# thimabru1010/ResUnet-a_mltsk_keras

Hardware: AMD Instinct MI355X
Metric: training patches/sec (256×256, 6-ch, bs=8/GPU) at 1/2/4/8 MI355X (higher is better)
Workload: dtype bf16; 1 GPU; cfg3: ResUnet-a d6 multitask (seg+bound+dist+color) Tanimoto-dual, 256x256x6, 6 classes, Adam, full train step (fwd+loss+bwd+allreduce+update); global_batch=8, per_gpu_batch=8, parallelism=dp1

## Files before the change

### include/rua_hip.h

```cpp
#ifndef RUA_HIP_H
#define RUA_HIP_H
#include <stdint.h>
#ifdef __cplusplus
extern "C" {
#endif

#define RUA_F32 0
#define RUA_BF16 1
#define RUA_MAX_SEG 6
#define RUA_MAX_BRANCH 4
#define RUA_MAX_WGRAD_BATCH 32
#define RUA_MAX_WGRAD_GROUP 8

#define RUA_OK 0
#define RUA_ERR_ARG (-1)
#define RUA_ERR_LAUNCH (-2)

int rua_version(void);
const char* rua_last_error(void);
int rua_device_info(int* cu_count, int* lds_bytes, char* arch, int arch_len);

typedef struct rua_conv_seg {
  const void* x;
  const void* w;
// ... 10 lines not shown
  float eps, momentum;
  const float* gamma; const float* beta;
  float* moving_mean; float* moving_var;
  float* scale; float* shift; float* mean; float* rstd;
} rua_bn_fold;

typedef struct rua_conv_desc {
  rua_conv_seg seg[RUA_MAX_SEG];
  int32_t nseg;
  int32_t N, H, W, Cout;
  int32_t stride;
  int32_t dtype;
  const float* bias;
  const void* aux;
  int32_t aux_mode;
  const float* mscale;
  const float* mshift;
  int32_t out_relu;
  int32_t accumulate;
  void* y;
  int32_t out_stride, OH, OW;
  double* stats;
  int32_t stats_mode;
  void* workspace;
  int64_t workspace_bytes;
  int32_t stats_replicas;
  const float* bias_more[3];
  const float* in_scale;
  const float* in_shift;
  int32_t in_relu;
  int32_t pad_fold;
  const struct rua_bn_fold* in_fold;
} rua_conv_desc;
int rua_conv_fwd(const rua_conv_desc* d, void* stream);
int rua_conv_fwd_group(const rua_conv_desc* d, int n, void* stream);
int rua_conv_group_last_grids(void);
int rua_conv_group_band_ok(const rua_conv_desc* d, int n);
int rua_conv_group_last_band(void);
int rua_conv_group_last_chain(void);
int rua_conv_fwd_sum(const rua_conv_desc* d, int n, void* stream);
int rua_conv_sum_last_kernel(void);
int rua_conv_sum_kernel(const rua_conv_desc* d, int n);
int rua_conv_smem_bytes(const rua_conv_desc* d);
int64_t rua_conv_workspace_bytes(const rua_conv_desc* d);
void* rua_prof_event_create(void);
int rua_prof_event_record(void* ev, void* hip_stream);
int rua_prof_event_elapsed_us(void* start, void* stop, double* us);
void rua_prof_event_destroy(void* ev);
void rua_profile_mid_event(void* hip_event);
int rua_profile_mid_event_fired(void);
int rua_conv_last_ksplit(void);
int rua_conv_tile_bn(const rua_conv_desc* d);
int rua_conv_kernel_id(const rua_conv_desc* d);
int rua_conv_fused_input_ok(const rua_conv_desc* d);
int rua_conv_tile_bm(const rua_conv_desc* d);

typedef struct rua_wgrad_desc {
  const void* a;  int32_t C, Hs, Ws;
  const void* dy; int32_t Cout, H, W;
  int32_t N, stride, dil, taps, dtype;
  float* dw;
  void* workspace;
  int64_t workspace_bytes;
  const float* in_scale;
  const float* in_shift;
  int32_t in_relu;
  int32_t defer;
  int32_t group_members;
  int32_t batch;
  const int32_t* overwrite_dev;
} rua_wgrad_desc;
typedef struct rua_wgrad_pending {
  int32_t kind;
  int32_t parts;
  int64_t n;
  const float* partials;
  float* dw;
  int32_t CC;
  int32_t blocks;
  int32_t block_begin, pad;
  const int32_t* overwrite_dev;
} rua_wgrad_pending;
int rua_wgrad_plan(const rua_wgrad_desc* d, rua_wgrad_pending* out);
int rua_wgrad_reduce_batch(const rua_wgrad_pending* items_dev, int n_items, int total_blocks, void* stream);
int rua_conv_wgrad(const rua_wgrad_desc* d, void* stream);
int rua_conv_wgrad_group(const rua_wgrad_desc* d, int n, void* stream);
int rua_wgrad_group_last_grids(void);
int rua_wgrad_group_plan(const rua_wgrad_desc* d, int n, rua_wgrad_pending* out);
int64_t rua_wgrad_workspace_bytes(const rua_wgrad_desc* d);
int rua_wgrad_kind(const rua_wgrad_desc* d);
int rua_wgrad_img_kind(const rua_wgrad_desc* d);

typedef struct rua_wprep_item { int64_t src_off, dst_off; int32_t taps, Cout, C, pad; } rua_wprep_item;
int rua_weight_prep(const float* master, void* w_fwd, void* w_dgrad, const rua_wprep_item* items_dev,
                    int n_items, int max_elems, int dtype, void* stream);
int rua_weight_prep_dgrad(const void* w_fwd, void* w_dgrad, const rua_wprep_item* items_dev, int n_items, int max_elems, const int32_t* blockmap_dev,
                          int n_blocks, int dtype, void* stream);
int rua_wprep_blocks(int taps, int Cout, int C);

int rua_stem_fwd(const float* x, const float* w, const float* b, void* y, int64_t M, int Cin, int Cout, int dtype, void* stream);
int rua_stem_fwd_stats(const float* x, const float* w, const float* b, void* y, int64_t M, int Cin, int Cout, int dtype, double* stats, int replicas, void* stream);
int rua_stem_bwd(const float* x, const void* dy, float* dw, float* db, int64_t M, int Cin, int Cout, int dtype, void* stream);
int rua_stem_fwd_pack(const float* x, const float* w, const float* b, void* y, int64_t M, int Cin, int Cout, int dtype, double* stats, int replicas,
                      void* xpack, void* stream);
int rua_stem_bwd_fold(float* tmp, float* dw, float* db, int Cin, int Cout, void* stream);
int rua_head_fwd(const void* x, const float* w, const float* b, float* z, float* p, int64_t M, int Cin, int Cout, int act, int dtype, void* stream);
// ... 176 lines not shown
```

### resunet_a_mltsk_keras_amd/_lib.py

```python
from __future__ import annotations

import ctypes as C
import os

HERE = os.path.dirname(os.path.abspath(__file__))
LIB_PATH = os.environ.get("RUA_LIB_PATH") or os.path.join(HERE, "librua_hip.so")

RUA_F32, RUA_BF16 = 0, 1
RUA_MAX_SEG, RUA_MAX_BRANCH, RUA_MAX_WGRAD_GROUP, RUA_MAX_WGRAD_BATCH = 6, 4, 8, 32
LOSS_TANIMOTO, LOSS_WCE, LOSS_CE_LOGITS, LOSS_BCE_LOGITS, LOSS_MSE = 0, 1, 2, 3, 4
ACT_NONE, ACT_SOFTMAX, ACT_SIGMOID = 0, 1, 2

vp, i32, i64, f32, f64 = C.c_void_p, C.c_int32, C.c_int64, C.c_float, C.c_double


class ConvSeg(C.Structure):
    _fields_ = [("x", vp), ("w", vp), ("C", i32), ("Hs", i32), ("Ws", i32), ("up_shift", i32), ("dil", i32), ("taps", i32)]


class ConvDesc(C.Structure):
    _fields_ = [("seg", ConvSeg * RUA_MAX_SEG), ("nseg", i32), ("N", i32), ("H", i32), ("W", i32), ("Cout", i32),
                ("stride", i32), ("dtype", i32), ("bias", vp), ("aux", vp), ("aux_mode", i32), ("mscale", vp),
                ("mshift", vp), ("out_relu", i32), ("accumulate", i32), ("y", vp), ("out_stride", i32), ("OH", i32),
                ("OW", i32), ("stats", vp), ("stats_mode", i32), ("workspace", vp), ("workspace_bytes", i64), ("stats_replicas", i32),
# ... 11 lines not shown
                ("in_scale", vp), ("in_shift", vp), ("in_relu", i32), ("defer", i32), ("group_members", i32), ("batch", i32), ("overwrite_dev", vp)]


class WgradPending(C.Structure):
    _fields_ = [("kind", i32), ("parts", i32), ("n", i64), ("partials", vp), ("dw", vp), ("CC", i32), ("blocks", i32),
                ("block_begin", i32), ("pad", i32), ("overwrite_dev", vp)]


class TaniHead(C.Structure):
    _fields_ = [("sums", vp), ("replicas", i32), ("B", i32), ("C", i32), ("grad_scale", f32), ("loss_out", vp), ("coef", vp), ("per_sample", vp)]


class DzHead(C.Structure):
    _fields_ = [("kind", i32), ("act", i32), ("p", vp), ("y", vp), ("coef", vp), ("class_w", vp), ("grad_scale", f32), ("B", i32), ("HW", i64),
                ("C", i32), ("pad", i32), ("dz", vp)]


class BnBranch(C.Structure):
    _fields_ = [("gamma", vp), ("beta", vp), ("moving_mean", vp), ("moving_var", vp), ("scale", vp), ("shift", vp),
                ("mean", vp), ("rstd", vp), ("out", vp), ("stats", vp), ("replicas", i32), ("pad", i32), ("out_stats", vp)]


class BnFwdDesc(C.Structure):
    _fields_ = [("x", vp), ("M", i64), ("C", i32), ("dtype", i32), ("nb", i32), ("relu", i32), ("training", i32), ("replicas", i32),
                ("stats", vp), ("count", f64), ("bessel_n", f64), ("momentum", f32), ("eps", f32), ("br", BnBranch * RUA_MAX_BRANCH)]


class BnBwdBranch(C.Structure):
    _fields_ = [("g", vp), ("stats2", vp), ("replicas", i32), ("stats2_out", i32), ("gamma", vp), ("mean", vp), ("rstd", vp),
                ("scale", vp), ("shift", vp), ("dgamma", vp), ("dbeta", vp)]


class BnBwdDesc(C.Structure):
    _fields_ = [("x", vp), ("dskip", vp), ("dx", vp), ("M", i64), ("C", i32), ("dtype", i32), ("nb", i32), ("masked", i32),
                ("accumulate", i32), ("pad", i32), ("count", f64), ("br", BnBwdBranch * RUA_MAX_BRANCH),
                ("skip_stats", vp), ("skip_replicas", i32), ("pad2", i32), ("dx_stats", vp), ("dx_replicas", i32), ("pad3", i32)]


class WprepItem(C.Structure):
    _fields_ = [("src_off", i64), ("dst_off", i64), ("taps", i32), ("Cout", i32), ("C", i32), ("pad", i32)]


PP = C.POINTER(vp)

_SIGS = {
    "rua_version": ([], i32),
    "rua_device_info": ([C.POINTER(i32), C.POINTER(i32), C.c_char_p, i32], i32),
    "rua_conv_fwd": ([C.POINTER(ConvDesc), vp], i32),
    "rua_conv_fwd_group": ([C.POINTER(ConvDesc), i32, vp], i32),
    "rua_conv_smem_bytes": ([C.POINTER(ConvDesc)], i32),
    "rua_conv_tile_bn": ([C.POINTER(ConvDesc)], i32),
    "rua_conv_tile_bm": ([C.POINTER(ConvDesc)], i32),
    "rua_conv_kernel_id": ([C.POINTER(ConvDesc)], i32),
    "rua_conv_fused_input_ok": ([C.POINTER(ConvDesc)], i32),
    "rua_conv_last_ksplit": ([], i32),
    "rua_conv_group_last_grids": ([], i32),
    "rua_conv_group_band_ok": ([C.POINTER(ConvDesc), i32], i32),
    "rua_conv_group_last_band": ([], i32),
    "rua_conv_group_last_chain": ([], i32),
    "rua_conv_fwd_sum": ([C.POINTER(ConvDesc), i32, vp], i32),
    "rua_conv_sum_last_kernel": ([], i32),
    "rua_conv_sum_kernel": ([C.POINTER(ConvDesc), i32], i32),
    "rua_conv_wgrad_group": ([C.POINTER(WgradDesc), i32, vp], i32),
    "rua_wgrad_group_last_grids": ([], i32),
    "rua_wgrad_group_plan": ([C.POINTER(WgradDesc), i32, C.POINTER(WgradPending)], i32),
    "rua_profile_mid_event": ([vp], None),
    "rua_profile_mid_event_fired": ([], i32),
    "rua_prof_event_create": ([], vp),
    "rua_prof_event_record": ([vp, vp], i32),
    "rua_prof_event_elapsed_us": ([vp, vp, C.POINTER(f64)], i32),
    "rua_prof_event_destroy": ([vp], None),
    "rua_graph_kernel_nodes": ([vp, C.POINTER(i32), C.POINTER(i32)], i32),
    "rua_conv_workspace_bytes": ([C.POINTER(ConvDesc)], i64),
    "rua_conv_wgrad": ([C.POINTER(WgradDesc), vp], i32),
    "rua_wgrad_workspace_bytes": ([C.POINTER(WgradDesc)], i64),
    "rua_wgrad_kind": ([C.POINTER(WgradDesc)], i32),
    "rua_wgrad_img_kind": ([C.POINTER(WgradDesc)], i32),
    "rua_wgrad_plan": ([C.POINTER(WgradDesc), C.POINTER(WgradPending)], i32),
    "rua_wgrad_reduce_batch": ([vp, i32, i32, vp], i32),
    "rua_weight_prep": ([vp, vp, vp, vp, i32, i32, i32, vp], i32),
    "rua_weight_prep_dgrad": ([vp, vp, vp, i32, i32, vp, i32, i32, vp], i32),
    "rua_wprep_blocks": ([i32, i32, i32], i32),
    "rua_stem_fwd": ([vp, vp, vp, vp, i64, i32, i32, i32, vp], i32),
    "rua_stem_fwd_stats": ([vp, vp, vp, vp, i64, i32, i32, i32, vp, i32, vp], i32),
    "rua_stem_bwd": ([vp, vp, vp, vp, i64, i32, i32, i32, vp], i32),
    "rua_stem_fwd_pack": ([vp, vp, vp, vp, i64, i32, i32, i32, vp, i32, vp, vp], i32),
    "rua_stem_bwd_fold": ([vp, vp, vp, i32, i32, vp], i32),
    "rua_head_fwd": ([vp, vp, vp, vp, vp, i64, i32, i32, i32, i32, vp], i32),
    "rua_head_fwd_loss": ([vp, vp, vp, vp, vp, vp, vp, vp, i32, i64, i32, i32, i32, i32, vp], i32),
    "rua_head_fwd_loss_rep": ([vp, vp, vp, vp, vp, vp, vp, i32, vp, i32, i64, i32, i32, i32, i32, vp], i32),
    "rua_head_bwd": ([vp, vp, vp, vp, i32, vp, vp, vp, i64, i64, i32, i32, i32, i32, vp], i32),
    "rua_head_bwd_sums": ([vp, vp, vp, vp, i32, vp, vp, vp, vp, i64, i64, i32, i32, i32, i32, vp], i32),
    "rua_col_stats": ([vp, i64, i32, vp, i32, i32, vp], i32),
    "rua_col_stats2": ([vp, vp, vp, vp, i32, i64, i32, vp, i32, i32, vp], i32),
    "rua_stats_replicas": ([i64], i32),
    "rua_bn_finalize": ([vp, i32, f64, f64, vp, vp, vp, vp, f32, f32, i32, vp, vp, vp, vp, i32, vp], i32),
    "rua_bn_apply": ([vp, i32, PP, PP, i32, PP, i64, i32, i32, vp], i32),
    "rua_bn_bwd_finalize": ([vp, i32, f64, vp, vp, vp, vp, vp, vp, vp, vp, i32, vp], i32),
    "rua_bn_bwd_apply": ([i32, PP, PP, PP, PP, PP, PP, i32, vp, vp, vp, i32, i64, i32, i32, vp], i32),
    "rua_stats_to_f32": ([vp, i32, i32, PP, i32, vp], i32),
    "rua_bn_fwd": ([C.POINTER(BnFwdDesc), vp], i32),
    "rua_bn_fwd_group": ([C.POINTER(BnFwdDesc), i32, vp], i32),
    "rua_bn_fwd_group_last_grids": ([], i32),
    "rua_bn_bwd": ([C.POINTER(BnBwdDesc), vp], i32),
    "rua_bn_bwd_group": ([C.POINTER(BnBwdDesc), i32, vp], i32),
    "rua_bn_bwd_group_last_grids": ([], i32),
# ... 116 lines not shown
```

### resunet_a_mltsk_keras_amd/csrc/capi.cpp

```cpp
#include <hip/hip_runtime.h>
#include <stdarg.h>
#include <stdio.h>
#include <string.h>
#include <stdint.h>
#include "common.h"

static thread_local char g_err[512] = "";
RuaTuning g_tune;

void rua_set_error(const char* fmt, ...) {
  va_list ap;
  va_start(ap, fmt);
  vsnprintf(g_err, sizeof(g_err), fmt, ap);
  va_end(ap);
}

extern "C" const char* rua_last_error(void) { return g_err; }
extern "C" int rua_version(void) { return 200; }

extern "C" int rua_device_info(int* cu_count, int* lds_bytes, char* arch, int arch_len) {
  hipDeviceProp_t prop;
  int dev = 0;
  if (hipGetDevice(&dev) != hipSuccess || hipGetDeviceProperties(&prop, dev) != hipSuccess) {
    rua_set_error("rua_device_info: no HIP device");
// ... 41 lines not shown
  int k = 0;
  if (n && hipGraphGetNodes((hipGraph_t)graph, nodes, &n) == hipSuccess)
    for (size_t i = 0; i < n; ++i) {
      hipGraphNodeType t;
      if (hipGraphNodeGetType(nodes[i], &t) == hipSuccess && t == hipGraphNodeTypeKernel) ++k;
    }
  delete[] nodes;
  if (kernels) *kernels = k;
  if (total) *total = (int)n;
  return RUA_OK;
}

int rua_device_index() {
  int dev = 0;
  if (hipGetDevice(&dev) != hipSuccess || dev < 0) { (void)hipGetLastError(); dev = 0; }
  return dev;
}

int rua_cu_count() {
  static int cached[64] = {0};
  const int dev = rua_device_index();
  if (dev >= 64) return 256;
  if (cached[dev] == 0) {
    int n = 0;
    if (hipDeviceGetAttribute(&n, hipDeviceAttributeMultiprocessorCount, dev) != hipSuccess || n <= 0) { (void)hipGetLastError(); n = 256; }
    cached[dev] = n;
  }
  int n = cached[dev] - (g_tune.cu_reserve > 0 ? g_tune.cu_reserve : 0);
  return n < 16 ? 16 : n;
}

struct TuneKey { const char* name; int* i; long long* ll; };
static const TuneKey* tune_table(int* n) {
  static const TuneKey t[] = {
    {"conv_force_bn", &g_tune.conv_force_bn, nullptr}, {"conv_force_bm", &g_tune.conv_force_bm, nullptr}, {"conv_dma", &g_tune.conv_dma, nullptr},
    {"conv_pw", &g_tune.conv_pw, nullptr}, {"conv_pw_minm", nullptr, &g_tune.conv_pw_minm}, {"conv_pw_blocks", &g_tune.conv_pw_blocks, nullptr},
    {"conv_halo", &g_tune.conv_halo, nullptr}, {"conv_dmap", &g_tune.conv_dmap, nullptr}, {"dmap_target", &g_tune.dmap_target, nullptr},
    {"dmap_fused_finish", &g_tune.dmap_fused_finish, nullptr}, {"dmap_rowb", &g_tune.dmap_rowb, nullptr}, {"dmap_bm64", &g_tune.dmap_bm64, nullptr},
    {"wgrad_pw", &g_tune.wgrad_pw, nullptr}, {"wgpw_blocks", &g_tune.wgpw_blocks, nullptr}, {"wgpw_r", &g_tune.wgpw_r, nullptr},
    {"wgd_blocks", &g_tune.wgd_blocks, nullptr}, {"wgrad_dmap", &g_tune.wgrad_dmap, nullptr}, {"wgd_mintiles", &g_tune.wgd_mintiles, nullptr},
    {"wgrad_blocks", &g_tune.wgrad_blocks, nullptr}, {"bn_grid", &g_tune.bn_grid, nullptr}, {"tani_vec", &g_tune.tani_vec, nullptr},
    {"metrics_blocks", &g_tune.metrics_blocks, nullptr}, {"stem_blocks", &g_tune.stem_blocks, nullptr}, {"head_blocks", &g_tune.head_blocks, nullptr},
    {"conv_img", &g_tune.conv_img, nullptr}, {"conv_strip", &g_tune.conv_strip, nullptr}, {"wgrad_slabs", &g_tune.wgrad_slabs, nullptr},
    {"strip_narrow_maxd", &g_tune.strip_narrow_maxd, nullptr}, {"conv_group", &g_tune.conv_group, nullptr}, {"wgrad_group", &g_tune.wgrad_group, nullptr},
    {"wgrad_batch_blocks", &g_tune.wgrad_batch_blocks, nullptr}, {"wgd_ks_slow", &g_tune.wgd_ks_slow, nullptr}, {"head_fwd2", &g_tune.head_fwd2, nullptr},
    {"head_fwd3", &g_tune.head_fwd3, nullptr}, {"head_fwd3_bpc", &g_tune.head_fwd3_bpc, nullptr}, {"stem_reg", &g_tune.stem_reg, nullptr},
    {"stats_blocks", &g_tune.stats_blocks, nullptr}, {"conv_band", &g_tune.conv_band, nullptr}, {"conv_band64", &g_tune.conv_band64, nullptr},
    {"conv_band64m", &g_tune.conv_band64m, nullptr}, {"strip_group_share", &g_tune.strip_group_share, nullptr}, {"band_dbg", &g_tune.band_dbg, nullptr},
    {"fill_kernel", &g_tune.fill_kernel, nullptr}, {"bn_regs", &g_tune.bn_regs, nullptr}, {"wgrad_taps_share", &g_tune.wgrad_taps_share, nullptr},
    {"dmap_chain", &g_tune.dmap_chain, nullptr}, {"epi_fast", &g_tune.epi_fast, nullptr}, {"dmap_spread", &g_tune.dmap_spread, nullptr},
    {"bn_bwd_group", &g_tune.bn_bwd_group, nullptr}, {"conv_small", &g_tune.conv_small, nullptr}, {"strip_stag", &g_tune.strip_stag, nullptr},
    {"cu_reserve", &g_tune.cu_reserve, nullptr}, {"wgrad_rows", &g_tune.wgrad_rows, nullptr}, {"strip_seglen", &g_tune.strip_seglen, nullptr},
    {"band_stag", &g_tune.band_stag, nullptr}, {"conv_band128m", &g_tune.conv_band128m, nullptr}, {"conv_img2", &g_tune.conv_img2, nullptr},
    {"dbg_ptr", nullptr, &g_tune.dbg_ptr},
  };
  *n = (int)(sizeof(t) / sizeof(t[0]));
  return t;
}
extern "C" int rua_set_tuning(const char* key, int64_t value) {
  int n; const TuneKey* t = tune_table(&n);
  for (int i = 0; key && i < n; ++i)
    if (strcmp(t[i].name, key) == 0) { if (t[i].i) *t[i].i = (int)value; else *t[i].ll = (long long)value; return RUA_OK; }
  rua_set_error("rua_set_tuning: unknown key '%s'", key ? key : "(null)");
  return RUA_ERR_ARG;
}
extern "C" int rua_get_tuning(const char* key, int64_t* value) {
  int n; const TuneKey* t = tune_table(&n);
  for (int i = 0; key && value && i < n; ++i)
    if (strcmp(t[i].name, key) == 0) { *value = t[i].i ? (int64_t)*t[i].i : (int64_t)*t[i].ll; return RUA_OK; }
  rua_set_error("rua_get_tuning: unknown key '%s'", key ? key : "(null)");
  return RUA_ERR_ARG;
}
extern "C" const char* rua_tuning_key(int index) {
  int n; const TuneKey* t = tune_table(&n);
  return (index >= 0 && index < n) ? t[index].name : nullptr;
}
```

### resunet_a_mltsk_keras_amd/csrc/common.h

```cpp
#pragma once
#include <hip/hip_runtime.h>
#include <stdint.h>
#include <stdio.h>
#include <string.h>
#include "../../include/rua_hip.h"

typedef __bf16 bf16_t;
typedef __attribute__((ext_vector_type(16))) float f32x16;
typedef __attribute__((ext_vector_type(4))) float f32x4;
typedef __attribute__((ext_vector_type(8))) __bf16 bf16x8;
typedef __attribute__((ext_vector_type(4))) short s16x4;

void rua_set_error(const char* fmt, ...);
#define RUA_CHECK_ARG(cond, ...) do { if (!(cond)) { rua_set_error(__VA_ARGS__); return RUA_ERR_ARG; } } while (0)
#define RUA_LAUNCH_CHECK(name) do { hipError_t e_ = hipGetLastError(); if (e_ != hipSuccess) { \
    rua_set_error("%s: %s", name, hipGetErrorString(e_)); return RUA_ERR_LAUNCH; } } while (0)

template <typename T> struct ET;
template <> struct ET<float> {
  static constexpr int VEC = 4;
  static __device__ __forceinline__ void unpack(const uint4& v, float* f) {
    f[0] = __uint_as_float(v.x); f[1] = __uint_as_float(v.y); f[2] = __uint_as_float(v.z); f[3] = __uint_as_float(v.w);
  }
  static __device__ __forceinline__ uint4 pack(const float* f) {
// ... 3 lines not shown
template <> struct ET<bf16_t> {
  static constexpr int VEC = 8;
  static __device__ __forceinline__ void unpack(const uint4& v, float* f) {
    f[0] = __uint_as_float(v.x << 16); f[1] = __uint_as_float(v.x & 0xffff0000u);
    f[2] = __uint_as_float(v.y << 16); f[3] = __uint_as_float(v.y & 0xffff0000u);
    f[4] = __uint_as_float(v.z << 16); f[5] = __uint_as_float(v.z & 0xffff0000u);
    f[6] = __uint_as_float(v.w << 16); f[7] = __uint_as_float(v.w & 0xffff0000u);
  }
  static __device__ __forceinline__ uint32_t pk(float a, float b) {
    typedef __attribute__((ext_vector_type(2))) __bf16 bf2;
    bf2 r; r[0] = (__bf16)a; r[1] = (__bf16)b;
    return __builtin_bit_cast(uint32_t, r);
  }
  static __device__ __forceinline__ uint4 pack(const float* f) {
    return make_uint4(pk(f[0], f[1]), pk(f[2], f[3]), pk(f[4], f[5]), pk(f[6], f[7]));
  }
};

__device__ __forceinline__ uint4 ldg16(const void* p) { return *reinterpret_cast<const uint4*>(p); }

typedef __attribute__((ext_vector_type(4))) unsigned int u32x4_t;
#define RUA_OOB 0xFFFFFFF0u
__device__ __forceinline__ __amdgpu_buffer_rsrc_t make_rsrc(const void* p, unsigned bytes) {
  return __builtin_amdgcn_make_buffer_rsrc(const_cast<void*>(p), 0, bytes, 0x00020000);
}
__device__ __forceinline__ uint4 bufload16(__amdgpu_buffer_rsrc_t r, unsigned byte_off) {
  const u32x4_t v = __builtin_amdgcn_raw_buffer_load_b128(r, byte_off, 0, 0);
  return make_uint4(v[0], v[1], v[2], v[3]);
}
__device__ __forceinline__ void stg16(void* p, const uint4& v) { *reinterpret_cast<uint4*>(p) = v; }

__device__ __forceinline__ float wave_sum(float v) {
#pragma unroll
  for (int o = 32; o > 0; o >>= 1) v += __shfl_xor(v, o, 64);
  return v;
}

struct RuaTuning {
  int conv_force_bn = 0, conv_force_bm = 0, conv_dma = -1, conv_pw = 1;
  long long conv_pw_minm = 65536;
  int conv_pw_blocks = 0, conv_halo = 1, conv_dmap = 1, dmap_target = 0, dmap_fused_finish = 0, dmap_rowb = 64, dmap_bm64 = 1;
  int wgrad_pw = 3 , wgpw_blocks = 0, wgpw_r = 0, wgd_blocks = 0, wgrad_dmap = 1, wgd_mintiles = 10 , wgrad_blocks = 0;
  int bn_grid = 0, tani_vec = 1, metrics_blocks = 0, stem_blocks = 0, head_blocks = 0;
  int conv_strip = 1, wgrad_slabs = 1, strip_narrow_maxd = 0, strip_group_share = 1;
  int conv_group = 63;
  int stats_blocks = 0;
  int stem_reg = 1;
  int head_fwd3 = 1;
  int head_fwd3_bpc = 0;
  int head_fwd2 = 1;
  int conv_img2 = 1;
  int conv_img = 0;
  int conv_small = 4096;
  int bn_bwd_group = 1;
  int dmap_spread = 1;
  int epi_fast = 1;
  int dmap_chain = 0;
  int wgrad_taps_share = 1;
  int bn_regs = 1;
  int fill_kernel = 1;
  int band_dbg = 0;
  int conv_band64m = 1;
  int conv_band64 = 1;
  long long dbg_ptr = 0;
  int conv_band128m = 13;
  int conv_band = 1;
  int wgd_ks_slow = 1;
  int wgrad_rows = 127;
  int cu_reserve = 0;
  int strip_seglen = 0;
  int band_stag = 1;
  int strip_stag = 1;
  int wgrad_group = 23;
  int wgrad_batch_blocks = 0;
};
extern RuaTuning g_tune;
int rua_cu_count();
int rua_device_index();
void rua_record_mid_event(hipStream_t st);
struct RuaPerDevFlag { bool f[64] = {}; bool& get() { return f[rua_device_index() & 63]; } };

__device__ __forceinline__ void replica_sum(const double* __restrict__ stats, int R, int C, int c, double& s1, double& s2) {
  double a1 = 0, a2 = 0, b1 = 0, b2 = 0;
  int r = 0;
  for (; r + 8 <= R; r += 8) {
    double x[8], y[8];
#pragma unroll
    for (int u = 0; u < 8; ++u) { x[u] = stats[(size_t)(r + u) * 2 * C + c]; y[u] = stats[(size_t)(r + u) * 2 * C + C + c]; }
    a1 += (x[0] + x[1]) + (x[2] + x[3]); b1 += (x[4] + x[5]) + (x[6] + x[7]);
    a2 += (y[0] + y[1]) + (y[2] + y[3]); b2 += (y[4] + y[5]) + (y[6] + y[7]);
  }
  for (; r + 4 <= R; r += 4) {
    const double x0 = stats[(size_t)(r + 0) * 2 * C + c], y0 = stats[(size_t)(r + 0) * 2 * C + C + c];
    const double x1 = stats[(size_t)(r + 1) * 2 * C + c], y1 = stats[(size_t)(r + 1) * 2 * C + C + c];
    const double x2 = stats[(size_t)(r + 2) * 2 * C + c], y2 = stats[(size_t)(r + 2) * 2 * C + C + c];
    const double x3 = stats[(size_t)(r + 3) * 2 * C + c], y3 = stats[(size_t)(r + 3) * 2 * C + C + c];
    a1 += x0 + x1; b1 += x2 + x3; a2 += y0 + y1; b2 += y2 + y3;
  }
  for (; r < R; ++r) { a1 += stats[(size_t)r * 2 * C + c]; a2 += stats[(size_t)r * 2 * C + C + c]; }
  s1 = a1 + b1; s2 = a2 + b2;
}

__device__ __forceinline__ float ld_f32_or_zero(const float* p, int c, int n) {
  return __builtin_bit_cast(float, __builtin_amdgcn_raw_buffer_load_b32(make_rsrc(p, p ? (unsigned)(n * 4) : 0u), (unsigned)(c * 4), 0, 0));
}

// ... 100 lines not shown
```

### resunet_a_mltsk_keras_amd/csrc/conv_mfma.hip

```cpp
#include "common.h"


template <typename T> __device__ __forceinline__ void load8(const unsigned char* base, size_t elem_off, float* f) {
  if constexpr (sizeof(T) == 2) {
    ET<T>::unpack(ldg16(base + elem_off * 2), f);
  } else {
    ET<T>::unpack(ldg16(base + elem_off * 4), f);
    ET<T>::unpack(ldg16(base + elem_off * 4 + 16), f + 4);
  }
}
template <typename T> __device__ __forceinline__ void store8(unsigned char* base, size_t elem_off, const float* f) {
  if constexpr (sizeof(T) == 2) {
    stg16(base + elem_off * 2, ET<T>::pack(f));
  } else {
    stg16(base + elem_off * 4, ET<T>::pack(f));
    stg16(base + elem_off * 4 + 16, ET<T>::pack(f + 4));
  }
}

template <typename T, int BM, int BN> __host__ __device__ constexpr int conv_smem_base() {
  constexpr int ROWB = (sizeof(T) == 2) ? 80 : 132;
  constexpr int a = 2 * (BM + BN) * ROWB;
  constexpr int b = BM * (BN + 4) * 4 + 4 * (BN / 8) * 16 * 4;
  return ((a > b ? a : b) + 15) / 16 * 16;
// ... 1701 lines not shown
      if (j < nstep) {
        a[j] = bufload16(rx, abase + (unsigned)((kk + j) * 32));
#pragma unroll
        for (int t = 0; t < BNT; ++t) b[t][j] = bufload16(rw, bbase[t] + (unsigned)((kk + j) * 32));
      }
#pragma unroll
    for (int j = 0; j < CH; ++j)
      if (j < nstep) {
#pragma unroll
        for (int t = 0; t < BNT; ++t)
          acc[t] = __builtin_amdgcn_mfma_f32_32x32x16_bf16(__builtin_bit_cast(bf16x8, a[j]), __builtin_bit_cast(bf16x8, b[t][j]), acc[t], 0, 0, 0);
      }
    ks += nstep; kk += nstep;
    if (kk == nk && ks < ke) { ++seg; kk = 0; enter(); }
  }
  float* mine = part + wid * BM * CSTR;
#pragma unroll
  for (int t = 0; t < BNT; ++t)
#pragma unroll
    for (int i = 0; i < 16; ++i) mine[((i & 3) + 8 * (i >> 2) + 4 * lh) * CSTR + t * 32 + lr] = acc[t][i];
  __syncthreads();
  for (int e = tid; e < BM * BN; e += 256) {
    const int r = e / BN, c = e - r * BN, o = r * CSTR + c;
    part[o] = ((part[o] + part[BM * CSTR + o]) + part[2 * BM * CSTR + o]) + part[3 * BM * CSTR + o];
  }
  __syncthreads();
  conv_epilogue<T, BM, BN>(p, m0, n0, bm_i, part, CSTR, sred);
}
template <int BNT> __global__ __launch_bounds__(256) void conv_small(const ConvK p) { conv_small_body<BNT>(p); }
template <int BNT> __global__ __launch_bounds__(256) void conv_small_g(const ConvKG g) {
  const ConvK& p = g.k[blockIdx.y];
  if ((int)blockIdx.x >= p.nbm * p.nbn) return;
  conv_small_body<BNT>(p);
}

static bool pick_small(const rua_conv_desc* d) {
  if (!g_tune.conv_small || d->dtype != RUA_BF16 || d->in_scale || d->in_fold) return false;
  const long long M = (long long)d->N * d->H * d->W;
  if (M > g_tune.conv_small || d->Cout < 32) return false;
  for (int s_ = 0; s_ < d->nseg; ++s_)
    if (d->seg[s_].taps != 1 || d->seg[s_].C % 16 != 0) return false;
  return true;
}
static int launch_conv_small(ConvK& k, hipStream_t st) {
  k.nbm = (int)((k.M + 31) / 32); k.nbn = (k.Cout + 63) / 64;
  k.ksplit = 1; k.stages_per_split = 0; k.ws = nullptr; k.cnt = nullptr;
  constexpr int smem = (4 * 32 * 68 + 4 * 8 * 16) * 4;
  if (g_conv_group && (g_tune.conv_group & 16)) {
    if (!g_conv_group->add(7, (unsigned)(k.nbm * k.nbn), smem, k)) { rua_set_error("rua_conv_fwd_group: more than %d captured members", RUA_MAX_BRANCH); return RUA_ERR_ARG; }
    return RUA_OK;
  }
  hipLaunchKernelGGL((conv_small<2>), dim3(k.nbm * k.nbn), dim3(256), smem, st, k);
  RUA_LAUNCH_CHECK("conv_small");
  return RUA_OK;
}

static thread_local int g_last_ksplit = 1;
extern "C" int rua_conv_last_ksplit(void) { return g_last_ksplit; }

extern "C" int rua_conv_fwd(const rua_conv_desc* d, void* stream) {
  RUA_CHECK_ARG(d && d->nseg >= 1 && d->nseg <= RUA_MAX_SEG, "rua_conv_fwd: nseg out of range");
  RUA_CHECK_ARG(d->dtype == RUA_F32 || d->dtype == RUA_BF16, "rua_conv_fwd: bad dtype");
  const int vec = d->dtype == RUA_BF16 ? 8 : 4;
  RUA_CHECK_ARG(d->Cout > 0 && d->Cout % 8 == 0, "rua_conv_fwd: Cout=%d must be a multiple of 8", d->Cout);
  RUA_CHECK_ARG(d->N > 0 && d->H > 0 && d->W > 0 && d->stride >= 1, "rua_conv_fwd: bad output grid");
  RUA_CHECK_ARG(d->y != nullptr, "rua_conv_fwd: null output");
  RUA_CHECK_ARG(d->out_stride >= 1 && d->OH >= (d->H - 1) * d->out_stride + 1 && d->OW >= (d->W - 1) * d->out_stride + 1,
                "rua_conv_fwd: output tensor smaller than the strided grid");
  RUA_CHECK_ARG((long long)d->N * d->H * d->W < (1ll << 31), "rua_conv_fwd: too many pixels");
  RUA_CHECK_ARG(d->aux_mode == 0 || d->aux != nullptr, "rua_conv_fwd: aux_mode without aux");
  RUA_CHECK_ARG(d->stats_mode == 0 || d->stats != nullptr, "rua_conv_fwd: stats_mode without stats");
  RUA_CHECK_ARG(d->stats_mode != 2 || d->aux != nullptr, "rua_conv_fwd: stats_mode 2 needs aux");
  ConvK k;
  k.nseg = d->nseg;
  int units = 0;
  for (int s = 0; s < d->nseg; ++s) {
    const rua_conv_seg& g = d->seg[s];
    RUA_CHECK_ARG(g.x && g.w, "rua_conv_fwd: null segment pointer");
    RUA_CHECK_ARG(g.C > 0 && g.C % vec == 0, "rua_conv_fwd: segment C=%d not a multiple of %d", g.C, vec);
    RUA_CHECK_ARG(g.taps == 1 || g.taps == 9, "rua_conv_fwd: taps must be 1 or 9");
    RUA_CHECK_ARG(g.up_shift >= 0 && g.up_shift <= 4 && g.dil >= 1, "rua_conv_fwd: bad up_shift/dil");
    RUA_CHECK_ARG((long long)(d->H - 1) * d->stride < ((long long)g.Hs << g.up_shift) &&
                  (long long)(d->W - 1) * d->stride < ((long long)g.Ws << g.up_shift),
                  "rua_conv_fwd: segment %d source %dx%d (up %d) too small for output %dx%d stride %d", s, g.Hs, g.Ws, g.up_shift, d->H, d->W, d->stride);
    RUA_CHECK_ARG((long long)d->N * g.Hs * g.Ws * g.C * 4 < (1ll << 31), "rua_conv_fwd: source tensor must stay below 2 GiB (32-bit offsets)");
    RUA_CHECK_ARG(g.up_shift == 0 || g.taps == 1, "rua_conv_fwd: nearest-upsampled sources are 1x1 only");
    RUA_CHECK_ARG((long long)g.taps * d->Cout * g.C * 4 < (1ll << 31), "rua_conv_fwd: weight block too large");
    SegK& o = k.seg[s];
    o.x = (const unsigned char*)g.x; o.w = (const unsigned char*)g.w;
    o.C = g.C; o.Hs = g.Hs; o.Ws = g.Ws; o.up = g.up_shift; o.dil = g.dil; o.taps = g.taps;
    o.nchunk = (g.C + 31) / 32; o.ubegin = units;
    o.xbytes = (unsigned)((size_t)d->N * g.Hs * g.Ws * g.C * (d->dtype == RUA_BF16 ? 2 : 4));
    o.wbytes = (unsigned)((size_t)g.taps * d->Cout * g.C * (d->dtype == RUA_BF16 ? 2 : 4));
    units += g.taps * o.nchunk;
  }
  k.nunits = units;
  RUA_CHECK_ARG(units <= RUA_MAX_UNITS, "rua_conv_fwd: K = %d units of 32 channels exceeds the unit-table capacity %d", units, RUA_MAX_UNITS);
  k.N = d->N; k.H = d->H; k.W = d->W; k.Cout = d->Cout; k.stride = d->stride;
  k.M = (long long)d->N * d->H * d->W;
  k.bias = d->bias; k.aux = (const unsigned char*)d->aux; k.aux_mode = d->aux_mode;
  for (int q = 0; q < 3; ++q) k.bias_more[q] = d->bias ? d->bias_more[q] : nullptr;
  k.mscale = d->mscale; k.mshift = d->mshift; k.out_relu = d->out_relu; k.accumulate = d->accumulate;
  k.y = (unsigned char*)d->y; k.out_stride = d->out_stride; k.OH = d->OH; k.OW = d->OW;
  k.stats = d->stats; k.stats_mode = d->stats_mode;
  k.stats_R = d->stats_replicas < 1 ? 1 : d->stats_replicas;
  RUA_CHECK_ARG((k.stats_R & (k.stats_R - 1)) == 0, "rua_conv_fwd: stats_replicas must be a power of two");
  k.in_scale = d->in_scale; k.in_shift = d->in_shift; k.in_relu = d->in_relu;
  k.epi_fast = g_tune.epi_fast;
  hipStream_t st = (hipStream_t)stream;
  if (rua_pick_strip(d)) {
    k.nbn = 1; k.nbm = 1; k.ksplit = 1; k.stages_per_split = 0; k.ws = nullptr; k.cnt = nullptr;
    g_last_ksplit = 1;
    return rua_launch_conv_strip(k, d, st);
  }
  RUA_CHECK_ARG(d->in_scale == nullptr && d->in_fold == nullptr, "rua_conv_fwd: in_scale / in_shift / in_fold (normalise on load) is not available for "
                                        "this shape: ask rua_conv_fused_input_ok() first");
  if (pick_halo(d)) {
    k.nbn = 1; k.nbm = 1; k.ksplit = 1; k.stages_per_split = 0; k.ws = nullptr; k.cnt = nullptr;
    g_last_ksplit = 1;
    return launch_conv_halo(k, d->seg[0].dil, st);
  }
  if (pick_pw(d)) {
    k.nbn = 1; k.nbm = 1; k.ksplit = 1; k.stages_per_split = 0; k.ws = nullptr; k.cnt = nullptr;
    g_last_ksplit = 1;
    const int ks = pw_steps(d);
    return ks <= 2 ? launch_conv_pw<2>(k, d, st) : ks <= 4 ? launch_conv_pw<4>(k, d, st) : launch_conv_pw<6>(k, d, st);
  }
  if (pick_small(d)) {
    g_last_ksplit = 1;
    return launch_conv_small(k, st);
  }
  if (const int img2_ks = rua_pick_img2(d)) {
    g_last_ksplit = img2_ks;
    return rua_launch_conv_img2(k, d, img2_ks, st);
  }
  if (!g_conv_group && rua_band128_sum_ok(d)) {
    g_last_ksplit = 1;
    return rua_launch_band128_sum(d, st);
  }
  if (const int img_ks = pick_img(d)) {
    g_last_ksplit = img_ks;
    return launch_conv_img(k, d, img_ks, st);
  }
  if (pick_dmap(d)) {
    const int target = g_tune.dmap_target > 0 ? g_tune.dmap_target : rua_cu_count();
    k.nbn = (d->Cout + 127) / 128;
    k.nbm = (int)((k.M + 127) / 128);
    const int nstages = units / 2;
    const long long tiles = (long long)k.nbm * k.nbn;
    int want = 1;
    const int fused = g_tune.dmap_fused_finish;
    const size_t ws_usable = d->workspace_bytes > 4096 ? (size_t)d->workspace_bytes - 4096 : 0;
    const long long slabs = d->workspace ? (long long)(ws_usable / ((size_t)k.M * d->Cout * sizeof(float))) : 0;
    k.cnt = (fused && d->workspace && tiles <= 1024) ? reinterpret_cast<int*>((char*)d->workspace + ws_usable) : nullptr;
    if (slabs >= 2 && tiles < target) {
      want = (int)((target + tiles - 1) / tiles);
      if (want > nstages / 4) want = nstages / 4;
      if (want > 32) want = 32;
      if (want > slabs) want = (int)slabs;
      if (want < 1) want = 1;
      if (tiles * 2 >= target && nstages <= 40) want = 1;
    }
    k.ws = (float*)d->workspace;
    k.stages_per_split = (nstages + want - 1) / want;
    k.ksplit = (nstages + k.stages_per_split - 1) / k.stages_per_split;
    g_last_ksplit = k.ksplit;
    const int rowb = g_tune.dmap_rowb == 128 ? 128 : 64;
    const int bm64 = g_tune.dmap_bm64;
    if (bm64 && k.ksplit == 1 && tiles < target && tiles * 2 >= target) {
      k.nbm = (int)((k.M + 63) / 64);
      return launch_conv_dmap<64, 128, 64>(k, st);
    }
    return rowb == 128 ? launch_conv_dmap<128, 128, 128>(k, st) : launch_conv_dmap<128, 128, 64>(k, st);
  }
  const int bn = pick_bn(d, k.M);
  int bm = pick_bm(d, k.M, bn);
  k.nbn = (d->Cout + bn - 1) / bn;
  int nbm = (int)((k.M + bm - 1) / bm);
  k.nbm = nbm;
  const int nstages = (units + 1) / 2;
// ... 64 lines not shown
    if (rc == RUA_OK) { g_group_last_grids = 1; g_group_last_band = 2; }
    return rc;
  }
  if (rua_band64m_ok(d, n)) {
    const int rc = rua_launch_band64m(d, n, st);
    if (rc == RUA_OK) { g_group_last_grids = 1; g_group_last_band = 1; }
    return rc;
  }
  if (n == 1 || !g_tune.conv_group) {
    for (int i = 0; i < n; ++i) { const int rc = rua_conv_fwd(d + i, stream); if (rc != RUA_OK) return rc; }
    return RUA_OK;
  }
  ConvGroupCapture cap;
  cap.n = 0;
  cap.members = n;
  PwGroupCapture pwc;
  pwc.n = 0;
  rua_strip_group_reset();
  g_conv_group = &cap;
  g_pw_group = (g_tune.conv_group & 32) ? &pwc : nullptr;
  int rc = RUA_OK;
  for (int i = 0; i < n && rc == RUA_OK; ++i) rc = rua_conv_fwd(d + i, stream);
  g_conv_group = nullptr;
  g_pw_group = nullptr;
  if (rc != RUA_OK) { rua_strip_group_reset(); return rc; }
  int grids = n - cap.n - pwc.n - rua_strip_group_pending();
  for (int dense = 0; dense < 2; ++dense) {
    PwKG<2> g; int m = 0; unsigned gx = 0;
    for (int i = 0; i < pwc.n; ++i) if ((int)pwc.dense[i] == dense) { g.k[m++] = pwc.k[i]; if ((unsigned)pwc.k[i].nblk > gx) gx = (unsigned)pwc.k[i].nblk; }
    if (m == 0) continue;
    for (int i = m; i < RUA_MAX_BRANCH; ++i) g.k[i] = g.k[0];
    if (m == 1) { if (dense) hipLaunchKernelGGL((conv_pw<2, true>), dim3(gx), dim3(256), 0, st, g.k[0]); else hipLaunchKernelGGL((conv_pw<2, false>), dim3(gx), dim3(256), 0, st, g.k[0]); }
    else if (dense) hipLaunchKernelGGL((conv_pw_g<2, true>), dim3(gx, m), dim3(256), 0, st, g);
    else hipLaunchKernelGGL((conv_pw_g<2, false>), dim3(gx, m), dim3(256), 0, st, g);
    RUA_LAUNCH_CHECK("conv_pw (group)");
    ++grids;
  }
  rc = rua_strip_group_flush(st, &grids);
  if (rc != RUA_OK) return rc;
  bool done[RUA_MAX_BRANCH] = {false};
  for (int i = 0; i < cap.n; ++i) {
    if (done[i]) continue;
    int idx[RUA_MAX_BRANCH], m = 0;
    if (cap.kind[i] == 7) {
      unsigned gmax = 0;
      for (int j = i; j < cap.n; ++j)
        if (!done[j] && cap.kind[j] == 7) { idx[m++] = j; done[j] = true; if (cap.grid[j] > gmax) gmax = cap.grid[j]; }
      if (m == 1) hipLaunchKernelGGL((conv_small<2>), dim3(cap.grid[idx[0]]), dim3(256), cap.smem[idx[0]], st, cap.k[idx[0]]);
      else { ConvKG g; for (int q = 0; q < m; ++q) g.k[q] = cap.k[idx[q]]; hipLaunchKernelGGL((conv_small_g<2>), dim3(gmax, m), dim3(256), cap.smem[idx[0]], st, g); }
      RUA_LAUNCH_CHECK("conv_small (group)");
      ++grids;
      continue;
    }
    for (int j = i; j < cap.n; ++j)
      if (!done[j] && cap.kind[j] == cap.kind[i] && cap.grid[j] == cap.grid[i] && cap.smem[j] == cap.smem[i]) { idx[m++] = j; done[j] = true; }
    const bool chain = m >= 2 && (cap.kind[i] == 1 || cap.kind[i] == 2) && (g_tune.dmap_chain & cap.kind[i]) && chain_ok(cap, idx, m);
    if (chain) g_group_last_chain = m;
    if (chain && cap.kind[i] == 1) rc = issue_chain(cap, idx, m, conv_dmap_chain<128, 128, 64>, conv_dmap_chain_smem<128, 128>(), 0, st);
    else if (chain) rc = issue_chain(cap, idx, m, conv_dmap_chain<64, 128, 64>, conv_dmap_chain_smem<64, 128>(), 1, st);
    else if (cap.kind[i] == 1) rc = issue_group<ConvKG>(cap, idx, m, conv_dmap<128, 128, 64>, conv_dmap_g<128, 128, 64>, conv_dmap_smem<128, 128>(), st, "conv_dmap (group)");
    else if (cap.kind[i] == 6) rc = issue_group<ConvKG>(cap, idx, m, conv_dmap_s<128, 128, 64>, conv_dmap_gs<128, 128, 64>, conv_dmap_smem<128, 128, 4>(), st, "conv_dmap_s (group)");
    else if (cap.kind[i] == 2) rc = issue_group<ConvKG>(cap, idx, m, conv_dmap<64, 128, 64>, conv_dmap_g<64, 128, 64>, conv_dmap_smem<64, 128>(), st, "conv_dmap (group)");
    else rc = issue_group<ConvKG>(cap, idx, m, conv_igemm<bf16_t, 256, 64>, conv_igemm_g<bf16_t, 256, 64>, conv_smem<bf16_t, 256, 64>(), st, "conv_igemm (group)");
    if (rc != RUA_OK) return rc;
    ++grids;
  }
  g_group_last_grids = grids;
  return RUA_OK;
}

extern "C" int64_t rua_conv_workspace_bytes(const rua_conv_desc* d) {
  if (!d) return 0;
  return (int64_t)d->N * d->H * d->W * d->Cout * (int64_t)sizeof(float);
}

extern "C" int rua_conv_tile_bn(const rua_conv_desc* d) {
  if (!d) return RUA_ERR_ARG;
  if (pick_dmap(d)) return 128;
  return pick_bn(d, (long long)d->N * d->H * d->W);
}
extern "C" int rua_conv_fused_input_ok(const rua_conv_desc* d) { return (d && rua_pick_strip(d)) ? 1 : 0; }

extern "C" int rua_conv_kernel_id(const rua_conv_desc* d) {
  if (!d) return RUA_ERR_ARG;
  if (rua_pick_strip(d)) return 5;
  if (pick_halo(d)) return 3;
  if (pick_pw(d)) return 4;
  if (pick_small(d)) return 6;
  if (rua_pick_img2(d)) return 8;
  if (!g_conv_group && rua_band128_sum_ok(d)) return 9;
  if (pick_img(d)) return 7;
  if (pick_dmap(d)) return 2;
  return pick_dma(d, pick_bn(d, (long long)d->N * d->H * d->W)) ? 1 : 0;
}
extern "C" int rua_conv_tile_bm(const rua_conv_desc* d) {
  if (!d) return RUA_ERR_ARG;
  const long long M = (long long)d->N * d->H * d->W;
  if (pick_dmap(d)) {
    const int target = g_tune.dmap_target > 0 ? g_tune.dmap_target : rua_cu_count();
    const int bm64 = g_tune.dmap_bm64;
    const long long tiles = ((M + 127) / 128) * ((d->Cout + 127) / 128);
    int units = 0;
    for (int i = 0; i < d->nseg; ++i) units += d->seg[i].taps * (d->seg[i].C / 32);
    const bool split = d->workspace && d->workspace_bytes > 4096 &&
                       (size_t)(d->workspace_bytes - 4096) / ((size_t)M * d->Cout * sizeof(float)) >= 2 && units / 2 > 40;
    return (bm64 && !split && tiles < target && tiles * 2 >= target) ? 64 : 128;
  }
  return pick_bm(d, M, pick_bn(d, M));
}
```

Baseline: 1350 patches/s.

## Add streaming pointwise-conv kernel with direct-to-LDS panel loads and counted waits

```diff
diff --git a/include/rua_hip.h b/include/rua_hip.h
--- a/include/rua_hip.h
+++ b/include/rua_hip.h
@@ -86,6 +86,7 @@
 int rua_conv_last_ksplit(void);
 int rua_conv_tile_bn(const rua_conv_desc* d);
 int rua_conv_kernel_id(const rua_conv_desc* d);
+int rua_conv_small_form(const rua_conv_desc* d);
 int rua_conv_fused_input_ok(const rua_conv_desc* d);
 int rua_conv_tile_bm(const rua_conv_desc* d);
 
diff --git a/resunet_a_mltsk_keras_amd/_lib.py b/resunet_a_mltsk_keras_amd/_lib.py
--- a/resunet_a_mltsk_keras_amd/_lib.py
+++ b/resunet_a_mltsk_keras_amd/_lib.py
@@ -87,6 +87,7 @@
     "rua_conv_tile_bn": ([C.POINTER(ConvDesc)], i32),
     "rua_conv_tile_bm": ([C.POINTER(ConvDesc)], i32),
     "rua_conv_kernel_id": ([C.POINTER(ConvDesc)], i32),
+    "rua_conv_small_form": ([C.POINTER(ConvDesc)], i32),
     "rua_conv_fused_input_ok": ([C.POINTER(ConvDesc)], i32),
     "rua_conv_last_ksplit": ([], i32),
     "rua_conv_group_last_grids": ([], i32),
diff --git a/resunet_a_mltsk_keras_amd/csrc/capi.cpp b/resunet_a_mltsk_keras_amd/csrc/capi.cpp
--- a/resunet_a_mltsk_keras_amd/csrc/capi.cpp
+++ b/resunet_a_mltsk_keras_amd/csrc/capi.cpp
@@ -117,7 +117,7 @@
     {"bn_bwd_group", &g_tune.bn_bwd_group, nullptr}, {"conv_small", &g_tune.conv_small, nullptr}, {"strip_stag", &g_tune.strip_stag, nullptr},
     {"cu_reserve", &g_tune.cu_reserve, nullptr}, {"wgrad_rows", &g_tune.wgrad_rows, nullptr}, {"strip_seglen", &g_tune.strip_seglen, nullptr},
     {"band_stag", &g_tune.band_stag, nullptr}, {"conv_band128m", &g_tune.conv_band128m, nullptr}, {"conv_img2", &g_tune.conv_img2, nullptr},
-    {"dbg_ptr", nullptr, &g_tune.dbg_ptr},
+    {"conv_stream", &g_tune.conv_stream, nullptr}, {"conv_stream_all", &g_tune.conv_stream_all, nullptr}, {"dbg_ptr", nullptr, &g_tune.dbg_ptr},
   };
   *n = (int)(sizeof(t) / sizeof(t[0]));
   return t;
diff --git a/resunet_a_mltsk_keras_amd/csrc/common.h b/resunet_a_mltsk_keras_amd/csrc/common.h
--- a/resunet_a_mltsk_keras_amd/csrc/common.h
+++ b/resunet_a_mltsk_keras_amd/csrc/common.h
@@ -79,6 +79,8 @@
   int conv_img2 = 1;
   int conv_img = 0;
   int conv_small = 4096;
+  int conv_stream = 4096;
+  int conv_stream_all = 0;
   int bn_bwd_group = 1;
   int dmap_spread = 1;
   int epi_fast = 1;
diff --git a/resunet_a_mltsk_keras_amd/csrc/conv_mfma.hip b/resunet_a_mltsk_keras_amd/csrc/conv_mfma.hip
--- a/resunet_a_mltsk_keras_amd/csrc/conv_mfma.hip
+++ b/resunet_a_mltsk_keras_amd/csrc/conv_mfma.hip
@@ -1777,6 +1777,161 @@
   }
   hipLaunchKernelGGL((conv_small<2>), dim3(k.nbm * k.nbn), dim3(256), smem, st, k);
   RUA_LAUNCH_CHECK("conv_small");
+  return RUA_OK;
+}
+
+#define RUA_STREAM_WAIT_CASE(n) case n: asm volatile("s_waitcnt vmcnt(" #n ")" ::: "memory"); break;
+__device__ __forceinline__ void stream_wait_vm(int n) {
+  switch (n) {
+    RUA_STREAM_WAIT_CASE(1) RUA_STREAM_WAIT_CASE(2) RUA_STREAM_WAIT_CASE(3) RUA_STREAM_WAIT_CASE(4) RUA_STREAM_WAIT_CASE(5)
+    RUA_STREAM_WAIT_CASE(6) RUA_STREAM_WAIT_CASE(7) RUA_STREAM_WAIT_CASE(8) RUA_STREAM_WAIT_CASE(9) RUA_STREAM_WAIT_CASE(10)
+    RUA_STREAM_WAIT_CASE(11) RUA_STREAM_WAIT_CASE(12) RUA_STREAM_WAIT_CASE(13) RUA_STREAM_WAIT_CASE(14) RUA_STREAM_WAIT_CASE(15)
+    default: asm volatile("s_waitcnt vmcnt(0)" ::: "memory"); break;
+  }
+}
+constexpr int STREAM_BM = 64, STREAM_BN = 64, STREAM_CAP = 32, STREAM_TAB = 2048;
+static_assert(STREAM_CAP >= 16 && STREAM_CAP <= 32, "a pass must hold the widest panel (or it never advances); the counted waits go up to 15 instructions per wave");
+__host__ __device__ __forceinline__ int stream_panel(int C, int c0) {
+  int rem = C - c0, pw = 16;
+  if (rem > 128) rem = 128;
+  while (pw * 8 > rem) pw >>= 1;
+  return pw;
+}
+template <int PW>
+__device__ __forceinline__ void stream_panel_mma(const unsigned char* pan, int ra, int rb, int lh, f32x16& acc) {
+  constexpr int SH = PW == 16 ? 0 : PW == 8 ? 1 : PW == 4 ? 2 : 3;
+  const unsigned char* pa = pan + ra * (PW * 16);
+  const unsigned char* pb = pan + (STREAM_BM + rb) * (PW * 16);
+  const int swa = (ra >> SH) & (PW - 1), swb = (rb >> SH) & (PW - 1);
+  bf16x8 a[PW / 2], b[PW / 2];
+#pragma unroll
+  for (int ks = 0; ks < PW / 2; ++ks) {
+    a[ks] = *reinterpret_cast<const bf16x8*>(pa + (((2 * ks + lh) ^ swa) << 4));
+    b[ks] = *reinterpret_cast<const bf16x8*>(pb + (((2 * ks + lh) ^ swb) << 4));
+  }
+#pragma unroll
+  for (int ks = 0; ks < PW / 2; ++ks) acc = __builtin_amdgcn_mfma_f32_32x32x16_bf16(a[ks], b[ks], acc, 0, 0, 0);
+}
+__device__ __forceinline__ void conv_stream_body(const ConvK& p) {
+  typedef bf16_t T;
+  constexpr int BM = STREAM_BM, BN = STREAM_BN, CSTR = BN + 4, CAP = STREAM_CAP;
+  constexpr unsigned OOB = 0x80000000u;
+  extern __shared__ __attribute__((aligned(16))) unsigned char smem[];
+  unsigned* rowoff = reinterpret_cast<unsigned*>(smem);
+  unsigned char* stage = smem + STREAM_TAB;
+  const int tid = threadIdx.x, lane = tid & 63, wv = __builtin_amdgcn_readfirstlane(tid >> 6);
+  const int lr = lane & 31, lh = lane >> 5;
+  const int nwg = p.nbm * p.nbn, bid = blockIdx.x;
+  const int xcd = bid & 7, q8 = nwg >> 3, r8 = nwg & 7;
+  const int job = (xcd < r8 ? xcd * (q8 + 1) : r8 * (q8 + 1) + (xcd - r8) * q8) + (bid >> 3);
+  const int bn_i = job % p.nbn, bm_i = job / p.nbn;
+  const long long m0 = (long long)bm_i * BM;
+  const int n0 = bn_i * BN;
+  {
+    const int row = tid & 63;
+    const long long m = m0 + row;
+    const bool av = m < p.M;
+    const int mm = av ? (int)m : 0, HW = p.H * p.W;
+    const int n = mm / HW, rem = mm - n * HW, h = rem / p.W, w = rem - h * p.W;
+    const int ah = h * p.stride, aw = w * p.stride;
+    for (int s_ = tid >> 6; s_ < p.nseg; s_ += 4) {
+      const SegK& sg = p.seg[s_];
+      rowoff[s_ * 64 + row] = av ? (unsigned)((((n * sg.Hs + (ah >> sg.up)) * sg.Ws + (aw >> sg.up)) * sg.C) * 2) : OOB;
+    }
+  }
+  __syncthreads();
+  f32x16 acc;
+#pragma unroll
+  for (int i = 0; i < 16; ++i) acc[i] = 0.f;
+  const int ra = (wv >> 1) * 32 + lr, rb = (wv & 1) * 32 + lr;
+  int seg = 0, c0 = 0;
+  while (seg < p.nseg) {
+    int s1 = seg, c1 = c0, used = 0;
+    while (s1 < p.nseg) {
+      const SegK& sg = p.seg[s1];
+      const int PW = stream_panel(sg.C, c1);
+      if (used + PW > CAP) break;
+      const int lg = 31 - __builtin_clz(PW), sh = 4 - lg;
+      const __amdgpu_buffer_rsrc_t rx = make_rsrc(sg.x, sg.xbytes), rw = make_rsrc(sg.w, sg.wbytes);
+      unsigned char* pan = stage + used * 2048;
+      for (int q = wv; q < 2 * PW; q += 4) {
+        const bool isa = q < PW;
+        const int row = ((q & (PW - 1)) << (6 - lg)) + (lane >> lg);
+        const int piece = (lane & (PW - 1)) ^ ((row >> sh) & (PW - 1));
+        const unsigned ch = (unsigned)((c1 + piece * 8) * 2);
+        if (isa) {
+          __builtin_amdgcn_raw_ptr_buffer_load_lds(rx, (lds_void_p)(pan + q * 1024), 16, rowoff[s1 * 64 + row] + ch, 0, 0, 0);
+        } else {
+          const int co = n0 + row;
+          __builtin_amdgcn_raw_ptr_buffer_load_lds(rw, (lds_void_p)(pan + q * 1024), 16, co < p.Cout ? (unsigned)(co * sg.C * 2) + ch : OOB, 0, 0, 0);
+        }
+      }
+      used += PW; c1 += PW * 8;
+      if (c1 == sg.C) { ++s1; c1 = 0; }
+    }
+    int done = 0;
+    while (seg != s1 || c0 != c1) {
+      const int C = p.seg[seg].C;
+      const int PW = stream_panel(C, c0);
+      const unsigned char* pan = stage + done * 2048;
+      done += PW;
+      stream_wait_vm((used - done) >> 1);
+      __builtin_amdgcn_s_barrier();
+      if (PW == 16) stream_panel_mma<16>(pan, ra, rb, lh, acc);
+      else if (PW == 8) stream_panel_mma<8>(pan, ra, rb, lh, acc);
+      else if (PW == 4) stream_panel_mma<4>(pan, ra, rb, lh, acc);
+      else stream_panel_mma<2>(pan, ra, rb, lh, acc);
+      c0 += PW * 8;
+      if (c0 == C) { ++seg; c0 = 0; }
+    }
+    asm volatile("s_waitcnt lgkmcnt(0)" ::: "memory");
+    __builtin_amdgcn_s_barrier();
+  }
+  float* tile = reinterpret_cast<float*>(stage);
+#pragma unroll
+  for (int i = 0; i < 16; ++i) tile[((wv >> 1) * 32 + (i & 3) + 8 * (i >> 2) + 4 * lh) * CSTR + (wv & 1) * 32 + lr] = acc[i];
+  __syncthreads();
+  conv_epilogue<T, BM, BN>(p, m0, n0, bm_i, tile, CSTR, tile + BM * CSTR);
+}
+__global__ __launch_bounds__(256) void conv_stream(const ConvK p) { conv_stream_body(p); }
+__global__ __launch_bounds__(256) void conv_stream_g(const ConvKG g) {
+  const ConvK& p = g.k[blockIdx.y];
+  if ((int)blockIdx.x >= p.nbm * p.nbn) return;
+  conv_stream_body(p);
+}
+
+static bool pick_stream(const rua_conv_desc* d) {
+  if (g_tune.conv_stream < 0 || d->dtype != RUA_BF16 || d->in_scale || d->in_fold || d->Cout < 32) return false;
+  const long long M = (long long)d->N * d->H * d->W;
+  if (M <= g_tune.conv_stream) return false;
+  if (M * d->Cout * 4 >= (1ll << 31) || (long long)d->N * d->OH * d->OW * d->Cout * 2 >= (1ll << 31)) return false;
+  for (int s_ = 0; s_ < d->nseg; ++s_)
+    if (d->seg[s_].taps != 1 || d->seg[s_].C % 16 != 0) return false;
+  if (g_tune.conv_stream_all) return true;
+  if (g_conv_group || d->nseg != 1 || d->seg[0].up_shift != 0 || d->stride != 1 || d->aux_mode != 0 || d->seg[0].C < 64) return false;
+  return M <= (d->stats_mode ? 8192 : 32768);
+}
+constexpr int STREAM_SMEM_MAX = STREAM_TAB + STREAM_CAP * 2048;
+static int launch_conv_stream(ConvK& k, hipStream_t st) {
+  k.nbm = (int)((k.M + STREAM_BM - 1) / STREAM_BM); k.nbn = (k.Cout + STREAM_BN - 1) / STREAM_BN;
+  k.ksplit = 1; k.stages_per_split = 0; k.ws = nullptr; k.cnt = nullptr;
+  int pieces = 0;
+  for (int s_ = 0; s_ < k.nseg; ++s_) pieces += k.seg[s_].C / 8;
+  if (pieces > STREAM_CAP) pieces = STREAM_CAP;
+  constexpr int epi = (STREAM_BM * (STREAM_BN + 4) + 4 * (STREAM_BN / 8) * 16) * 4;
+  const int smem = STREAM_TAB + (pieces * 2048 > epi ? pieces * 2048 : epi);
+  static RuaPerDevFlag attr;
+  if (!attr.get()) {
+    (void)hipFuncSetAttribute(reinterpret_cast<const void*>(&conv_stream), hipFuncAttributeMaxDynamicSharedMemorySize, STREAM_SMEM_MAX);
+    (void)hipFuncSetAttribute(reinterpret_cast<const void*>(&conv_stream_g), hipFuncAttributeMaxDynamicSharedMemorySize, STREAM_SMEM_MAX);
+    attr.get() = true;
+  }
+  if (g_conv_group && (g_tune.conv_group & 16)) {
+    if (!g_conv_group->add(5, (unsigned)(k.nbm * k.nbn), smem, k)) { rua_set_error("rua_conv_fwd_group: more than %d captured members", RUA_MAX_BRANCH); return RUA_ERR_ARG; }
+    return RUA_OK;
+  }
+  hipLaunchKernelGGL(conv_stream, dim3(k.nbm * k.nbn), dim3(256), smem, st, k);
+  RUA_LAUNCH_CHECK("conv_stream");
   return RUA_OK;
 }
 
@@ -1851,6 +2006,10 @@
     const int ks = pw_steps(d);
     return ks <= 2 ? launch_conv_pw<2>(k, d, st) : ks <= 4 ? launch_conv_pw<4>(k, d, st) : launch_conv_pw<6>(k, d, st);
   }
+  if (pick_stream(d)) {
+    g_last_ksplit = 1;
+    return launch_conv_stream(k, st);
+  }
   if (pick_small(d)) {
     g_last_ksplit = 1;
     return launch_conv_small(k, st);
@@ -2021,6 +2180,16 @@
       ++grids;
       continue;
     }
+    if (cap.kind[i] == 5) {
+      unsigned gmax = 0; int smax = 0;
+      for (int j = i; j < cap.n; ++j)
+        if (!done[j] && cap.kind[j] == 5) { idx[m++] = j; done[j] = true; if (cap.grid[j] > gmax) gmax = cap.grid[j]; if (cap.smem[j] > smax) smax = cap.smem[j]; }
+      if (m == 1) hipLaunchKernelGGL(conv_stream, dim3(gmax), dim3(256), smax, st, cap.k[idx[0]]);
+      else { ConvKG g; for (int q = 0; q < m; ++q) g.k[q] = cap.k[idx[q]]; hipLaunchKernelGGL(conv_stream_g, dim3(gmax, m), dim3(256), smax, st, g); }
+      RUA_LAUNCH_CHECK("conv_stream (group)");
+      ++grids;
+      continue;
+    }
     for (int j = i; j < cap.n; ++j)
       if (!done[j] && cap.kind[j] == cap.kind[i] && cap.grid[j] == cap.grid[i] && cap.smem[j] == cap.smem[i]) { idx[m++] = j; done[j] = true; }
     const bool chain = m >= 2 && (cap.kind[i] == 1 || cap.kind[i] == 2) && (g_tune.dmap_chain & cap.kind[i]) && chain_ok(cap, idx, m);
@@ -2055,12 +2224,16 @@
   if (rua_pick_strip(d)) return 5;
   if (pick_halo(d)) return 3;
   if (pick_pw(d)) return 4;
-  if (pick_small(d)) return 6;
+  if (pick_stream(d) || pick_small(d)) return 6;
   if (rua_pick_img2(d)) return 8;
   if (!g_conv_group && rua_band128_sum_ok(d)) return 9;
   if (pick_img(d)) return 7;
   if (pick_dmap(d)) return 2;
   return pick_dma(d, pick_bn(d, (long long)d->N * d->H * d->W)) ? 1 : 0;
+}
+extern "C" int rua_conv_small_form(const rua_conv_desc* d) {
+  if (!d || rua_conv_kernel_id(d) != 6) return -1;
+  return pick_stream(d) ? 1 : 0;
 }
 extern "C" int rua_conv_tile_bm(const rua_conv_desc* d) {
   if (!d) return RUA_ERR_ARG;
```

After: 1353 patches/s, median of 6. Within noise of the previous version (+0.2%).
